# rust-bio/rust-bio

Measured on AMD Instinct MI355X. Metric: GCUPS (SW) + FM-index queries/sec, higher is better.
Workload: dtype int16; 1 GPU; 1000000 x 150 bp synthetic read pairs per GPU, Aligner::local affine-gap (-5,-1,+1,-1), score+coords+traceback ops (BASELINE configs[1]); pairs_per_gpu=1000000, read_len=150, parallelism=shard1

## Files before the change

### rust-bio_amd/csrc/sw_fill_pk16.inc

```
#include <type_traits>

#include "sw_kernels.h"

#ifndef PK16_CELL_KO
#define PK16_CELL_KO 0
#endif

namespace bgsw {
namespace pk16 {

typedef uint32_t pk;

typedef short s16x2 __attribute__((ext_vector_type(2)));
typedef unsigned short u16x2 __attribute__((ext_vector_type(2)));
typedef _Float16 h16x2 __attribute__((ext_vector_type(2)));
__device__ __forceinline__ s16x2 as_s(pk v) { return __builtin_bit_cast(s16x2, v); }
__device__ __forceinline__ u16x2 as_u(pk v) { return __builtin_bit_cast(u16x2, v); }
__device__ __forceinline__ pk bits(s16x2 v) { return __builtin_bit_cast(pk, v); }
__device__ __forceinline__ pk bits(u16x2 v) { return __builtin_bit_cast(pk, v); }
__device__ __forceinline__ pk pk_adds(pk a, pk b) { return bits(__builtin_elementwise_add_sat(as_s(a), as_s(b))); }
__device__ __forceinline__ pk pk_max(pk a, pk b) { return bits(__builtin_elementwise_max(as_s(a), as_s(b))); }
__device__ __forceinline__ pk pk_max3h(pk a, pk b, pk c) {
    const h16x2 x = __builtin_bit_cast(h16x2, a), y = __builtin_bit_cast(h16x2, b), z = __builtin_bit_cast(h16x2, c);
    return __builtin_bit_cast(pk, __builtin_elementwise_maximum(__builtin_elementwise_maximum(x, y), z));
}
__device__ __forceinline__ pk pk_min(pk a, pk b) { return bits(__builtin_elementwise_min(as_s(a), as_s(b))); }
__device__ __forceinline__ pk pk_add_u16(pk a, pk b) { return bits((u16x2)(as_u(a) + as_u(b))); }
__device__ __forceinline__ pk pk_sub_u16(pk a, pk b) { return bits((u16x2)(as_u(a) - as_u(b))); }
__device__ __forceinline__ pk pk_subs_u16(pk a, pk b) { return bits(__builtin_elementwise_sub_sat(as_u(a), as_u(b))); }
__device__ __forceinline__ pk pk_mad_u16(pk a, pk b, pk c) { return bits((u16x2)(as_u(a) * as_u(b) + as_u(c))); }
__device__ __forceinline__ pk dup16(int32_t v) { return ((uint32_t)v & 0xffffu) | ((uint32_t)v << 16); }
__device__ __forceinline__ pk bfi(pk mask, pk a, pk b) { return (a & mask) | (b & ~mask); }
__device__ __forceinline__ pk nz_mask(pk v, pk one) { return pk_sub_u16(pk_subs_u16(one, v), one); }

template <int LP>
__device__ __forceinline__ void scan_first_max(int ll, int64_t& v, uint32_t& idx) {
#pragma unroll
    for (int off = 1; off < LP; off <<= 1) {
        const int64_t ov = __shfl_up(v, off, LP);
        const uint32_t oi = (uint32_t)__shfl_up((int)idx, off, LP);
        if (ll >= off && !(v > ov)) {
            v = ov;
            idx = oi;
        }
    }
}

constexpr int32_t kFloor16 = -2048;

enum { CZ = 0, CF = 1, CI = 2 };
template <int R, int LP, int MODE, int XP, int XS, int YP, int YS, bool LF = false, int FR = 0>
__device__ __forceinline__ void sw_fill_pk16_body(const SwArgs& a) {
    constexpr bool FAST = MODE == 0;
    constexpr int PW = 64 / LP;
    constexpr int NW = tb_words(R);
    constexpr int NH = (R + 2) / 3;
    constexpr bool NARROW = true, LOCAL = XP == CZ && XS == CZ && YP == CZ && YS == CZ;
    constexpr bool ROW0_ZERO = YP == CZ && YS == CZ;
    constexpr int SH = 4;
    constexpr int32_t NEGS = kFloor16 * 16;
    constexpr pk CLEAN = 0xfff0fff0u, FLOORK = 0x80008000u, ONE = 0x00010001u;
    static_assert(LP == 16 || LP == 32, "lanes per pair");
    static_assert(R >= 1 && R <= 12, "rows per lane");
    static_assert(!LF || LOCAL, "LF is a flavour of the local kernel");
    static_assert(FR >= 0 && FR <= 2 && (!FR || LF), "the frame is a cell of the LF flavour");
    (void)NARROW;
    (void)LOCAL;
    constexpr int kTileStride = 20;
    constexpr int kParkDw = 64 * (4 * R + NH + 1), kTileDw = 2 * 64 * kTileStride;
    constexpr int kWaveDw = kParkDw > kTileDw ? kParkDw : kTileDw;
    __shared__ __align__(16) pk s_lds[4 * kWaveDw];
    pk* const wave_lds = s_lds + (threadIdx.x >> 6) * kWaveDw;

    const int lane = threadIdx.x & 63;
    const uint32_t wv = blockIdx.x * (blockDim.x >> 6) + (threadIdx.x >> 6);
    if ((uint64_t)wv * 2 * PW >= a.n_pairs) return;
    if (MODE == 2 && a.len_stats && a.len_stats[0] == a.len_stats[2] && a.len_stats[1] == a.len_stats[3]) return;
    const int g = lane / LP, ll = lane % LP;
    const SwScoring sc = a.sc;
    const SwGeom geo = a.g;
    auto scl = [](int32_t v) -> int32_t { return max(v, kFloor16) * 16; };
    const int32_t go_s = sc.go * 16, xs_s = sc.xs <= kFloor16 ? -(1 << 30) : sc.xs * 16;
    (void)xs_s;
    constexpr int32_t K_XS = C_XS << 1, K_MATCH = C_MATCH << 1, K_SUBST = C_SUBST << 1, K_INS = C_INS << 1,
                      K_DEL = C_DEL << 1, K_XP = C_XP << 1;
    constexpr pk NOFLAG = 0xfffefffeu;
    const pk GE = dup16(sc.ge * 16);
    const pk GOT_I = dup16(sc.go * 16 + K_INS + 1), GOT_D = dup16(sc.go * 16 + K_DEL + 1);
    const pk MISK = dup16((sc.mismatch * 16) | K_SUBST);
    const pk DELTA = dup16(((sc.match * 16) | K_MATCH) - ((sc.mismatch * 16) | K_SUBST));
    const pk XS16 = dup16(scl(sc.xs)), YS16 = dup16(scl(sc.ys));
    const pk XSCAP = sc.xs <= kFloor16 ? FLOORK : 0x7fff7fffu, YSCAP = sc.ys <= kFloor16 ? FLOORK : 0x7fff7fffu;
    (void)XS16; (void)YS16; (void)XSCAP; (void)YSCAP;
    const pk MISC = dup16(-((sc.mismatch * 16) | K_SUBST));
    (void)MISC;
    auto fr = [](int32_t c) -> pk { return (uint32_t)c * 0x10001u; };
    const int32_t gF = -16 * sc.ge, BF = pk16_frame_bias(sc);
    const pk GF = fr(gF);
    const pk KGOI = fr(sc.go * 16 + K_INS + 1 + gF), KGOD = fr(sc.go * 16 + K_DEL + 1 + gF);
    const pk KSUB = fr(((sc.mismatch * 16) | K_SUBST) + 2 * gF);
    const pk KREB = fr(gF * (R - 1));
    (void)GF; (void)KGOI; (void)KGOD; (void)KSUB; (void)KREB;
    constexpr bool DFLOOR = FR == 2 && !(PK16_CELL_KO & 1);
    constexpr bool SYMHI = FR == 2 && !(PK16_CELL_KO & 2);
    constexpr bool ROWMAX2 = FR == 2 && !(PK16_CELL_KO & 4);
    constexpr int SYM_SH = SYMHI ? 8 : 0;
    pk C16 = dup16(16), C32 = dup16(32), C1024 = dup16(1024);
    asm volatile("" : "+s"(C16), "+s"(C32), "+s"(C1024));

    const uint32_t pA = (2 * wv) * PW + g, pB = (2 * wv + 1) * PW + g;
    const bool okA = pA < a.n_pairs, okB = pB < a.n_pairs;
    uint32_t mA = 0, nA = 0, mB = 0, nB = 0;
    uint64_t xoA = 0, yoA = 0, xoB = 0, yoB = 0;
    const uint32_t* perm = a.slot_perm();
    if (okA) {
        const uint64_t r = a.pair0 + (perm ? perm[pA] : pA);
        xoA = a.x_off[r];
        yoA = a.y_off[r];
        mA = (uint32_t)(a.x_off[r + 1] - xoA);
        nA = (uint32_t)(a.y_off[r + 1] - yoA);
        if (len_over(geo, mA, nA)) mA = nA = 0;
    }
    if (okB) {
        const uint64_t r = a.pair0 + (perm ? perm[pB] : pB);
        xoB = a.x_off[r];
        yoB = a.y_off[r];
        mB = (uint32_t)(a.x_off[r + 1] - xoB);
        nB = (uint32_t)(a.y_off[r + 1] - yoB);
        if (len_over(geo, mB, nB)) mB = nB = 0;
    }
    const bool same = okA && okB && mA == mB && nA == nB;
    const bool two = okA && okB && !same;
    const bool m_last0 = LF || __all(!okA || mA % R == 0);
    if (MODE == 0 && !m_last0) return;
    if (MODE == 1 && m_last0) return;
    if (MODE == 2 && !__any(two)) return;
    const uint64_t job_words = tb_job_words(geo.nstrips, geo.nsteps, NW);

    auto do_pass = [&](const int pass) {
        const bool pair_ok = pass == 0 ? okA : two;
        const uint32_t P0 = pass == 0 ? pA : pB, P1 = (pass == 0 && !same) ? pA : pB;
        const uint32_t m = !pair_ok ? 0 : (pass == 0 ? mA : mB), n = !pair_ok ? 0 : (pass == 0 ? nA : nB);
        const uint64_t xs0 = pass == 0 ? xoA : xoB, ys0 = pass == 0 ? yoA : yoB;
        const uint64_t xs1 = (pass == 0 && !same) ? xoA : xoB, ys1 = (pass == 0 && !same) ? yoA : yoB;
        const uint8_t* x0 = a.x + xs0;
        const uint8_t* x1 = a.x + xs1;
        const bool packed = a.packed != 0;
        auto y_pair = [&](uint32_t col) -> pk {
            if (packed) return (sym2(a.y, ys0 + col) | (sym2(a.y, ys1 + col) << 16)) << SYM_SH;
            return ((uint32_t)a.y[ys0 + col] | ((uint32_t)a.y[ys1 + col] << 16)) << SYM_SH;
        };
        const uint32_t Q0 = pair_ok ? P0 : 0, Q1 = pair_ok ? P1 : 0;
        uint32_t* tb0 = (uint32_t*)a.tb + (size_t)(Q0 / PW) * job_words + ((Q0 % PW) * LP + ll) * 16u;
        uint32_t* tb1 = (uint32_t*)a.tb + (size_t)(Q1 / PW) * job_words + ((Q1 % PW) * LP + ll) * 16u;
        int32_t* aux0 = a.aux + (size_t)Q0 * geo.aux_stride;
        int32_t* aux1 = a.aux + (size_t)Q1 * geo.aux_stride;
        int32_t* gLx0 = aux0 + geo.off_Lx();
        int32_t* gLx1 = aux1 + geo.off_Lx();

        uint32_t m_w = m, n_w = n;
#pragma unroll
        for (int o = 32; o; o >>= 1) {
            m_w = max(m_w, (uint32_t)__shfl_xor((int)m_w, o));
            n_w = max(n_w, (uint32_t)__shfl_xor((int)n_w, o));
        }
        (void)m_w;
        n_w = (uint32_t)__builtin_amdgcn_readfirstlane((int)n_w);
        const uint32_t nsteps_w = n_w ? n_w + LP - 1 : 0;

        int32_t fold0;
        uint32_t lx0;
        col0_fold(sc, m, fold0, lx0);
        int32_t Sn0 = sc.ys;
        uint32_t Ly0 = n;
        int32_t S0n = 0;
        uint32_t sb0n = (ROW0_ZERO && n) ? row0_cell(sc, n).sbits : (uint32_t)TB_START;
        if (pair_ok && ll == 0) {
            const int32_t v = m ? (int32_t)col0_cell(sc, m, m, fold0).sbits : (int32_t)TB_START;
            aux0[0] = v;
            aux1[0] = v;
            if (m == 0) {
                if (LP == 16) {
                    *(uint8_t*)gLx0 = (uint8_t)lx0;
                    *(uint8_t*)gLx1 = (uint8_t)lx0;
                } else {
                    *(uint16_t*)gLx0 = (uint16_t)lx0;
                    *(uint16_t*)gLx1 = (uint16_t)lx0;
                }
            }
        }

        const uint32_t rb = (uint32_t)ll * R;
        const int32_t mrow = (int32_t)m - (int32_t)rb - 1;
        pk Sl[R], Dl[R], Il[R], SnR[R], SnB[R], Ly[R], px[R];
        uint64_t nib0S = 0, nib0I = 0;
        uint64_t xw0 = 0, xw1 = 0;
        if (packed && pair_ok && rb < m) {
            const uint32_t* p0 = (const uint32_t*)a.x + ((xs0 + rb) >> 4);
            const uint32_t* p1 = (const uint32_t*)a.x + ((xs1 + rb) >> 4);
            xw0 = (((uint64_t)p0[1] << 32) | p0[0]) >> (2 * ((uint32_t)(xs0 + rb) & 15u));
            xw1 = (((uint64_t)p1[1] << 32) | p1[0]) >> (2 * ((uint32_t)(xs1 + rb) & 15u));
        }
#pragma unroll
        for (int r = 0; r < R; r++) {
            const uint32_t i = rb + r + 1;
            px[r] = 0;
            Sl[r] = Dl[r] = Il[r] = SnR[r] = SnB[r] = FLOORK;
            Ly[r] = 0;
            if (pair_ok && i <= m) {
                px[r] = packed ? (((uint32_t)(xw0 >> (2 * r)) & 3u) | (((uint32_t)(xw1 >> (2 * r)) & 3u) << 16))
                               : ((uint32_t)x0[i - 1] | ((uint32_t)x1[i - 1] << 16));
                px[r] <<= SYM_SH;
                const Col0 c = col0_cell(sc, i, m, fold0);
                Sl[r] = dup16(scl(c.S));
                Il[r] = dup16(scl(c.I) | K_INS);
                nib0S |= (uint64_t)c.sbits << (4 * r);
                nib0I |= (uint64_t)c.ibits << (4 * r);
                if (YS != CI && c.S + sc.ys > NEG) {
                    SnR[r] = dup16(scl(c.S + sc.ys));
                    Ly[r] = dup16((int32_t)n);
                }
            }
        }
        pk diag0 = dup16((pair_ok && rb < m) ? scl(col0_S(sc, rb, m, fold0)) : NEGS);
        if (FR) {
            const int32_t off0 = BF + gF * ((int32_t)ll - 1);
#pragma unroll
            for (int r = 0; r < R; r++) {
                const pk o = fr(off0 + gF * r);
                Sl[r] = (pair_ok && rb + r + 1 <= m) ? Sl[r] + o : o;
                Il[r] += o;
                Dl[r] = 0;
            }
            diag0 = fr(off0 - gF) + ((pair_ok && rb < m) ? dup16(scl(col0_S(sc, rb, m, fold0))) : 0u);
        }

        pk S_out = FLOORK, I_out = FLOORK, cm_out = FLOORK, ca_out = 0, q_out = 0;
        pk ychunk = 0, ychunk_nx = 0;
        pk hwlast[NH];
#pragma unroll
        for (int k = 0; k < NH; k++) hwlast[k] = 0;
        pk lx_n = dup16((int32_t)lx0);
        pk* tileA = wave_lds + (0 * 64 + lane) * kTileStride;
        pk* tileB = wave_lds + (1 * 64 + lane) * kTileStride;
        uint32_t lxaccA = lx0 << (LP == 16 ? 24 : 16), lxaccB = lxaccA;
        if (pair_ok && (uint32_t)ll < n) ychunk_nx = y_pair((uint32_t)ll);

        auto merge_rows = [&](uint32_t blockbase) {
            const pk lybase = dup16((int32_t)(n - blockbase - 16u + (uint32_t)ll));
#pragma unroll
            for (int r = 0; r < R; r++) {
                const pk nr = pk_max(SnR[r], SnB[r] & CLEAN);
                const pk msk = nz_mask(nr ^ SnR[r], ONE);
                Ly[r] = bfi(msk, pk_add_u16(lybase, SnB[r] & 0x000f000fu), Ly[r]);
                SnR[r] = nr;
                SnB[r] = FLOORK;
            }
        };

        constexpr uint32_t tsteps = tb_tile_steps(NW);
        auto store_tile = [&](uint32_t s_any) {
            if (!pair_ok) return;
            const uint32_t off = (s_any / tsteps) * 1024u;
#pragma unroll
            for (int k = 0; k < 4; k++) {
                *(uint4*)&tb0[off + 4 * k] = *(const uint4*)&tileA[4 * k];
                *(uint4*)&tb1[off + 4 * k] = *(const uint4*)&tileB[4 * k];
            }
        };
        uint32_t s_all = pair_ok ? n + (uint32_t)ll : 0u;
#pragma unroll
        for (int o = 32; o; o >>= 1) s_all = min(s_all, (uint32_t)__shfl_xor((int)s_all, o));
        s_all = (uint32_t)__builtin_amdgcn_readfirstlane((int)s_all);
        auto run_steps = [&](auto mr_tag) {
        constexpr int MRk = decltype(mr_tag)::value;
        auto step = [&](auto allon_tag, auto fast_tag, auto trip_tag, const uint32_t s) {
            constexpr bool ALLON = decltype(allon_tag)::value;
            constexpr int TRIP = decltype(trip_tag)::value;
            static_assert(!TRIP || (ALLON && ROWMAX2), "trips are pairs of unpredicated steps of the FR == 2 cell");
            constexpr bool FB = decltype(fast_tag)::value;
            constexpr bool FOLD = XS != CI && !FB;
            if ((s & (LP - 1)) == 0) {
                ychunk = ychunk_nx;
                const uint32_t nb = s + LP + ll;
                if (pair_ok && nb < n) ychunk_nx = y_pair(nb);
            }
            pk S_up = (pk)wave_shr1((int)S_out, (int)S_out), I_up = (pk)wave_shr1((int)I_out, (int)I_out);
            if (FR) {
                S_up -= KREB;
                I_up -= KREB;
            }
            pk cm = FLOORK, ca = 0;
            if (FOLD) {
                cm = (pk)wave_shr1((int)cm_out, (int)cm_out);
                ca = (pk)wave_shr1((int)ca_out, (int)ca_out);
            }
            pk q = (pk)wave_shr1((int)q_out, (int)q_out);
            const uint32_t j = s + 1 - (uint32_t)ll;
            const bool col_ok = ALLON || (pair_ok && (j - 1) < n);
            const pk F0 = fr(BF + gF * (int32_t)s);
            (void)F0;
            if (ll == 0) {
                q = ychunk;
                S_up = FR ? F0 - GF : 0u;
                I_up = FR ? 0u : FLOORK;
                cm = FLOORK;
                ca = 0;
                if (!ROW0_ZERO && col_ok) {
                    const Row0 c = row0_cell(sc, j);
                    int32_t S0 = c.S;
                    uint32_t sb = c.sbits;
                    if (j == n && Sn0 > S0) {
                        S0 = Sn0;
                        sb = TB_YCLIP_SUFFIX;
                    } else if (S0 + sc.ys > Sn0) {
                        Sn0 = S0 + sc.ys;
                        Ly0 = n - j;
                    }
                    S0n = S0;
                    sb0n = sb;
                    S_up = dup16(scl(S0));
                }
            }
            ychunk = (pk)wave_shl1((int)ychunk, (int)ychunk);

            if (col_ok) {
                const pk sprio = dup16((int32_t)(15u - (s & 15u)));
                pk diag = diag0;
                diag0 = S_up;
                pk hw[NH];
                const pk ca_in = ca;
                pk cmk = cm | 0x000f000fu;
                pk snap = cmk;
                pk XKEY = dup16(K_XP);
                if (XP == CF || (XP == CZ && YP != CZ))
                    XKEY = dup16(scl(sc.xp + max(sc.yp, sc.go + sc.ge * ((int32_t)j - 1))) | K_XP);
#pragma unroll
                    for (int r = 0; r < R; r++) {
                        const bool maybe_m = MRk < 0 || r == MRk;
                        const bool is_m = MRk < 0 ? (r == mrow) : (r == MRk && mrow == MRk);
                        const pk e = pk_subs_u16(SYMHI ? DELTA : ONE, px[r] ^ q);
                        const pk Fr = F0 + (uint32_t)r * GF;
                        (void)Fr;
                        pk dk = diag + KSUB;
                        if (SYMHI && !(PK16_CELL_KO & 8)) asm("" : "+v"(dk));
                        const pk m_key = SYMHI   ? e + dk
                                         : FR == 2 ? pk_mad_u16(e, DELTA, diag) + KSUB
                                         : FR    ? pk_max(pk_mad_u16(e, DELTA, diag) + KSUB, Fr)
                                         : LF    ? pk_subs_u16(pk_mad_u16(e, DELTA, diag), MISC)
                                                 : pk_adds(diag, pk_mad_u16(e, DELTA, MISK));
                        const pk Iv_t = FR ? pk_max(I_up, S_up + KGOI) : pk_max(pk_adds(I_up, GE), pk_adds(S_up, GOT_I));
                        const pk Dv_t = DFLOOR ? pk_max3h(Dl[r], Sl[r] + KGOD, Fr)
                                        : FR   ? pk_max(Dl[r], Sl[r] + KGOD)
                                               : pk_max(pk_adds(Dl[r], GE), pk_adds(Sl[r], GOT_D));
                        const pk Iv = Iv_t & NOFLAG, Dv = Dv_t & NOFLAG;
                        pk kb = DFLOOR ? m_key : FR == 2 ? pk_max3h(m_key, Fr, Dv_t) : pk_max(m_key, Dv_t);
                        if (XP != CI && !LF) kb = pk_max(kb, XKEY);
                        kb = DFLOOR ? pk_max3h(kb, Dv_t, Iv_t) : FR == 2 ? pk_max3h(kb, Iv_t, Iv_t) : pk_max(kb, Iv_t);
                        if (FOLD && maybe_m)
                            kb = pk_max(kb, is_m ? ((cmk & CLEAN) | (0x00010001u * K_XS)) : FLOORK);
                        const pk best = kb & CLEAN;
                        const pk best_prev = Sl[r];
                        diag = Sl[r];
                        Sl[r] = best;
                        Dl[r] = Dv;
                        Il[r] = Iv;
                        S_up = best;
                        I_up = Iv;
                        if (FOLD) {
                            if (maybe_m) snap = is_m ? cmk : snap;
                            const pk fv = XS == CZ ? best : pk_min(pk_adds(best, XS16), XSCAP);
                            cmk = pk_max(cmk, fv | (0x00010001u * (uint32_t)(14 - r)));
                        }
                        if (YS != CI) {
                            const pk t1 = YS == CZ ? best : pk_min(pk_adds(best, YS16), YSCAP);
                            if (TRIP == 2)
                                SnB[r] = pk_max3h(SnB[r], best_prev - (Fr - GF - sprio - ONE), best - (Fr - sprio));
                            else if (TRIP == 0)
                                SnB[r] = pk_max(SnB[r], FR ? best - (Fr - sprio) : t1 | sprio);
                        }
                        const pk c5 = pk_mad_u16(Dv_t & ONE, C16, (kb & 0x000e000eu) | (Iv_t & ONE));
                        if (r % 3 == 0)
                            hw[r / 3] = c5;
                        else
                            hw[r / 3] = pk_mad_u16(c5, r % 3 == 1 ? C32 : C1024, hw[r / 3]);
                    }
                if (FOLD) {
                    const pk mbase = dup16(mrow - 14);
                    const pk lo = cmk & 0x000f000fu, slo = snap & 0x000f000fu;
                    if (mrow >= 0 && mrow < R) {
                        const pk is15 = nz_mask(slo ^ 0x000f000fu, ONE);
                        lx_n = bfi(is15, pk_add_u16(slo, mbase), ca_in);
                        if (LP == 16) {
                            lxaccA = __builtin_amdgcn_perm(lx_n, lxaccA, 0x04030201u);
                            lxaccB = __builtin_amdgcn_perm(lx_n, lxaccB, 0x06030201u);
                            if ((j & 3u) == 3u || j == n) {
                                const uint32_t sh = 8u * (3u - (j & 3u));
                                ((uint32_t*)gLx0)[j >> 2] = lxaccA >> sh;
                                ((uint32_t*)gLx1)[j >> 2] = lxaccB >> sh;
                            }
                        } else {
                            lxaccA = __builtin_amdgcn_perm(lx_n, lxaccA, 0x05040302u);
                            lxaccB = __builtin_amdgcn_perm(lx_n, lxaccB, 0x07060302u);
                            if ((j & 1u) == 1u || j == n) {
                                const uint32_t sh = 16u * (1u - (j & 1u));
                                ((uint32_t*)gLx0)[j >> 1] = lxaccA >> sh;
                                ((uint32_t*)gLx1)[j >> 1] = lxaccB >> sh;
                            }
                        }
                    }
                    {
                        const pk is15 = nz_mask(lo ^ 0x000f000fu, ONE);
                        ca = bfi(is15, pk_add_u16(lo, mbase), ca_in);
                    }
                    cm = cmk & CLEAN;
                }
                constexpr pk INV = 0x00010001u * (17u | (17u << 5) | (17u << 10));
                constexpr pk INV_LAST = 0x00010001u * ((R % 3 == 0) ? (17u | (17u << 5) | (17u << 10))
                                                      : (R % 3 == 1) ? 17u : (17u | (17u << 5)));
#pragma unroll
                for (int k = 0; k < NH; k++) {
                    hw[k] ^= (k == NH - 1) ? INV_LAST : INV;
                    hwlast[k] = hw[k];
                }
                const pk h0 = hw[0], h1 = NH > 1 ? hw[NH > 1 ? 1 : 0] : 0u;
                const uint32_t slot = (s % tsteps) * NW;
                if (NW == 1) {
                    tileA[slot] = __builtin_amdgcn_perm(h1, h0, 0x05040100u);
                    tileB[slot] = __builtin_amdgcn_perm(h1, h0, 0x07060302u);
                } else {
                    const pk h2 = hw[NH > 2 ? 2 : 0], h3 = NH > 3 ? hw[NH > 3 ? 3 : 0] : 0u;
                    *(uint2*)&tileA[slot] = make_uint2(__builtin_amdgcn_perm(h1, h0, 0x05040100u),
                                                       __builtin_amdgcn_perm(h3, h2, 0x05040100u));
                    *(uint2*)&tileB[slot] = make_uint2(__builtin_amdgcn_perm(h1, h0, 0x07060302u),
                                                       __builtin_amdgcn_perm(h3, h2, 0x07060302u));
                }
                S_out = S_up;
                I_out = I_up;
                if (FOLD) {
                    cm_out = cm;
                    ca_out = ca;
                }
                q_out = q;
            }
            if (s % tsteps == tsteps - 1) store_tile(s);
            if (YS != CI && (s & 15u) == 15u) merge_rows(s & ~15u);
        };
        uint32_t s = 0;
        const uint32_t s_on = min((uint32_t)(LP - 1), nsteps_w), s_off = max(s_on, min(s_all, nsteps_w));
        constexpr std::false_type no{};
        constexpr std::true_type yes{};
        constexpr std::bool_constant<LF> fast{};
        constexpr std::integral_constant<int, 0> single{};
        constexpr std::integral_constant<int, ROWMAX2 ? 1 : 0> first{};
        constexpr std::integral_constant<int, ROWMAX2 ? 2 : 0> second{};
        for (; s < s_on; s++) step(no, fast, single, s);
        if (ROWMAX2 && (s & 1u) && s < s_off) step(yes, fast, single, s++);
        for (; s + 1 < s_off; s += 2) {
            step(yes, fast, first, s);
            step(yes, fast, second, s + 1);
        }
        for (; s < s_off; s++) step(yes, fast, single, s);
        for (; s < nsteps_w; s++) step(no, fast, single, s);
        };
        run_steps(std::integral_constant<int, (FAST && !LF) ? R - 1 : -1>{});
        if (nsteps_w % tsteps) store_tile(nsteps_w - 1);
        if (YS != CI && nsteps_w) merge_rows((nsteps_w - 1) & ~15u);

        pk* park = wave_lds + lane;
        const pk offl = FR ? fr(BF + gF * ((int32_t)ll + (int32_t)n - 1)) : 0u;
#pragma unroll
        for (int r = 0; r < R; r++) {
            park[(0 * R + r) * 64] = FR ? Sl[r] - (offl + (uint32_t)r * GF) : Sl[r];
            park[(1 * R + r) * 64] = FR ? Il[r] - (offl + (uint32_t)r * GF) : Il[r];
            park[(2 * R + r) * 64] = SnR[r];
            park[(3 * R + r) * 64] = Ly[r];
        }
#pragma unroll
        for (int k = 0; k < NH; k++) park[(4 * R + k) * 64] = hwlast[k];
        park[(4 * R + NH) * 64] = lx_n;
        const int nhalf = (pair_ok && P1 != P0) ? 2 : 1;
        const int nhalf_w = __any(nhalf == 2) ? 2 : 1;
#pragma unroll 1
        for (int h = 0; h < nhalf_w; h++) {
            if (h >= nhalf) continue;
            const uint32_t hs = 16u * (uint32_t)h;
            int32_t* aux = h ? aux1 : aux0;
            int32_t* gLy = aux + geo.off_Ly();
            uint8_t* gBits = (uint8_t*)(aux + geo.off_bits());
            const uint32_t strip = 0;
            struct HalfS {
                const pk* p;
                uint32_t hs;
                __device__ int32_t operator[](int r) const { return (int32_t)(int16_t)(p[r * 64] >> hs); }
            };
            struct HalfU {
                const pk* p;
                uint32_t hs;
                __device__ uint32_t operator[](int r) const { return (p[r * 64] >> hs) & 0xffffu; }
            };
            int32_t Sl_u[R];
#pragma unroll
            for (int r = 0; r < R; r++) Sl_u[r] = (int32_t)(int16_t)(park[r * 64] >> hs);
            const HalfS Il_u{park + 1 * R * 64, hs}, Sn_u{park + 2 * R * 64, hs};
            const HalfU Ly_u{park + 3 * R * 64, hs};
            const uint32_t lx_n_u = (park[(4 * R + NH) * 64] >> hs) & 0xffffu;
            int64_t e_carry = INT64_MIN;
            uint32_t sbf_carry = TB_START, sb2_carry = TB_START;
            int64_t c1v = INT64_MIN, c2v = INT64_MIN;
            uint32_t c1i = 0, c2i = 0;
            auto cell_of = [&](int r) -> uint32_t {
                const uint32_t c = (park[(4 * R + r / 3) * 64] >> (hs + 5 * (r % 3))) & 31u;
                const uint32_t mv = (c >> 1) & 7u;
                return ((LF && mv == 0) ? (uint32_t)C_XP : mv) | ((c & 1u) << 3) | (c & 16u);
            };
            {
                constexpr bool EPI_FOLD_PRE = LF;
                int32_t(&Sl)[R] = Sl_u;
                const HalfS& Il = Il_u;
                const HalfS& Sn = Sn_u;
                const HalfU& Ly = Ly_u;
                const uint32_t lx_n = lx_n_u;
#include "sw_epilogue.inc"
            }
        }
    };
    do_pass(MODE == 2 ? 1 : 0);
}

template <int R, int LP, int XP, int XS, int YP, int YS, bool LF, int FR = 0>
__global__ __launch_bounds__(256) __attribute__((amdgpu_waves_per_eu(R <= 10 ? 3 : 2, R <= 10 ? 3 : 2))) void sw_fill_pk16_kernel(const SwArgs a) {
    sw_fill_pk16_body<R, LP, 0, XP, XS, YP, YS, LF, FR>(a);
}
template <int R, int LP, int XP, int XS, int YP, int YS, bool LF, int FR = 0>
__global__ __launch_bounds__(256) __attribute__((amdgpu_waves_per_eu(R <= 10 ? 3 : 2, R <= 10 ? 3 : 2))) void sw_fill_pk16_rest_kernel(const SwArgs a) {
    sw_fill_pk16_body<R, LP, 1, XP, XS, YP, YS, LF, FR>(a);
}
template <int R, int LP, int XP, int XS, int YP, int YS, bool LF, int FR = 0>
__global__ __launch_bounds__(256) __attribute__((amdgpu_waves_per_eu(R <= 10 ? 3 : 2, R <= 10 ? 3 : 2))) void sw_fill_pk16_second_kernel(const SwArgs a) {
    sw_fill_pk16_body<R, LP, 2, XP, XS, YP, YS, LF, FR>(a);
}

}
}

#define BG_PK16_CASE(LP_, R_)                                                                          \
    if (lp == LP_ && r == R_)                                                                         \
        return which == 0   ? pk16::sw_fill_pk16_kernel<R_, LP_, XP_, XS_, YP_, YS_, LF_, FR_>        \
               : which == 1 ? pk16::sw_fill_pk16_rest_kernel<R_, LP_, XP_, XS_, YP_, YS_, LF_, FR_>   \
                            : pk16::sw_fill_pk16_second_kernel<R_, LP_, XP_, XS_, YP_, YS_, LF_, FR_>;
```

### rust-bio_amd/csrc/sw_traceback.hip

```cpp
#include "sw_kernels.h"

namespace bgsw {

constexpr uint32_t kSegStride = 20;

template <int NW, bool PERM>
__global__ __launch_bounds__(256) __attribute__((amdgpu_waves_per_eu(5, 5))) void sw_traceback_kernel(const SwArgs a) {
    const uint32_t slot = blockIdx.x * blockDim.x + threadIdx.x;
    if (slot >= (a.n_eff ? a.n_eff[PERM ? 1 : 0] : a.n_pairs)) return;
    const uint32_t pair = PERM ? a.perm[slot] : slot;
    const SwScoring sc = a.sc;
    const SwGeom geo = a.g;
    const uint32_t R = geo.r, LP = geo.lp, PW = 64 / geo.lp;

    const uint64_t xo = a.x_off[a.pair0 + pair], yo = a.y_off[a.pair0 + pair];
    const uint32_t m = (uint32_t)(a.x_off[a.pair0 + pair + 1] - xo);
    const uint32_t n = (uint32_t)(a.y_off[a.pair0 + pair + 1] - yo);
    if (len_over(geo, m, n)) {
        bg_alignment_t bad = {};
        bad.xlen = m;
        bad.ylen = n;
        bad.ops_off = (a.pair0 + pair + 1) * a.ops_stride;
        bad.mode = (uint8_t)a.mode;
        bad.status = (int8_t)BG_ERR_INVALID_ARG;
        a.out[a.pair0 + pair] = bad;
        return;
    }

    const int32_t* aux = a.aux + (size_t)slot * geo.aux_stride;
    const int32_t* gLy = aux + geo.off_Ly();
    const int32_t* gLx = aux + geo.off_Lx();
    const uint8_t* bits = (const uint8_t*)(aux + geo.off_bits());
    const uint32_t sbits_m0 = (uint32_t)aux[0];
    const int32_t score = aux[1];
    const uint32_t lxn = (uint32_t)aux[2];

    const uint32_t job = slot / PW, grp = slot % PW;
    const uint32_t* tbj = (const uint32_t*)a.tb + (size_t)job * tb_job_words(geo.nstrips, geo.nsteps, NW);
    __shared__ __align__(16) uint32_t s_seg[256 * kSegStride];
    uint32_t* seg = s_seg + threadIdx.x * kSegStride;
    uint64_t seg_tag = ~0ull;
    auto cell = [&](uint32_t i, uint32_t j) -> uint32_t {
        const uint32_t i1 = i - 1, lrow = __umulhi(i1, geo.r_inv), rr = i1 - lrow * R;
        const uint32_t st = lrow >> geo.lp_shift, llc = lrow & (LP - 1);
        const uint64_t g = (uint64_t)st * geo.nsteps + (j - 1 + llc);
        constexpr uint32_t tsteps = 16 / NW;
        const uint64_t base = (g / tsteps) * 1024ull + (grp * LP + llc) * 16u;
        if (base != seg_tag) {
#pragma unroll
            for (int q = 0; q < 4; q++) *(uint4*)&seg[4 * q] = *(const uint4*)&tbj[base + 4 * q];
            seg_tag = base;
        }
        const uint32_t w = seg[(uint32_t)(g % tsteps) * NW + rr / 6];
        const uint32_t c = rr % 6;
        if (geo.tb_fmt == TBF_K1) return (w >> (5 * c)) & 31u;
        if (geo.tb_fmt == TBF_K1_LF) {
            const uint32_t u = (w >> (5 * c)) & 31u;
            return ((u >> 1) & 7u) | ((~u & 1u) << 3) | (~u & 16u);
        }
        const uint32_t v = (w >> (5 * (c % 3) + 16 * (c / 3))) & 31u;
        const uint32_t mv = (v >> 1) & 7u;
        return ((geo.tb_fmt == TBF_K1P_LF && mv == 0) ? (uint32_t)C_XP : mv) | ((v & 1u) << 3) | (v & 16u);
    };
    auto s_fill = [&](uint32_t i, uint32_t j) -> uint32_t {
        if (j == 0) {
            if (i == 0) return TB_START;
            if (i == m) return sbits_m0;
            return col0_cell(sc, i, m, NEG).sbits;
        }
        if (i == 0) return row0_cell(sc, j).sbits;
        return s_nibble_of_code(cell(i, j) & 7u);
    };
    auto s_nib = [&](uint32_t i, uint32_t j) -> uint32_t {
        if (j == n) return (uint32_t)bits[i] & 15u;
        return s_fill(i, j);
    };
    auto i_nib = [&](uint32_t i, uint32_t j) -> uint32_t {
        if (j == n) return (uint32_t)bits[i] >> 4;
        if (i == 0) return TB_START;
        if (j == 0) return col0_cell(sc, i, m, NEG).ibits;
        return (cell(i, j) & 8u) ? TB_INS : s_fill(i - 1, j);
    };
    auto d_nib = [&](uint32_t i, uint32_t j) -> uint32_t {
        if (j == 0) return TB_START;
        if (i == 0) return row0_cell(sc, j).dbits;
        return (cell(i, j) & 16u) ? TB_DEL : s_fill(i, j - 1);
    };

    uint8_t* ops_end = a.ops ? a.ops + (a.pair0 + pair + 1) * a.ops_stride : nullptr;
    uint32_t n_ops = 0;
    uint32_t clip_len[4] = {0, 0, 0, 0};
    uint32_t n_clips = 0;
    int status = BG_OK;
    const bool dword_ok = ops_end && (((uintptr_t)ops_end & 3) == 0);
    uint32_t acc = 0;
    auto push = [&](uint32_t op) {
        ++n_ops;
        if (!ops_end) return;
        if (dword_ok) {
            acc = (acc << 8) | op;
            if ((n_ops & 3) == 0) *(uint32_t*)(ops_end - n_ops) = acc;
        } else {
            ops_end[-(int64_t)n_ops] = (uint8_t)op;
        }
    };
    auto push_clip = [&](uint32_t op, uint32_t len) {
        if (a.filter_clips) return;
        if (n_clips < 4) clip_len[n_clips] = len;
        else status = BG_ERR_TRACEBACK;
        n_clips++;
        push(op);
    };

    uint32_t i = m, j = n;
    uint32_t xstart = 0, ystart = 0, xend = m, yend = n;
    uint32_t layer = s_nib(m, n);
    const uint32_t guard = 2 * (m + n) + 16;
    uint32_t c_here = 0;
    bool have_c = false;
    for (uint32_t steps = 0; layer != TB_START; steps++) {
        if (steps > guard || (ops_end && n_ops + 1 > a.ops_stride)) {
            status = BG_ERR_TRACEBACK;
            break;
        }
        if (layer >= TB_INS && layer <= TB_MATCH && i >= 1 && i <= m && j >= 1 && j < n) {
            const bool is_ins = layer == TB_INS, is_del = layer == TB_DEL;
            const uint32_t ti = i - (is_del ? 0u : 1u), tj = j - (is_ins ? 0u : 1u);
            if (ti >= 1 && tj >= 1) {
                if (!have_c && (is_ins || is_del)) c_here = cell(i, j);
                const bool ext = (is_ins && (c_here & 8u)) || (is_del && (c_here & 16u));
                push(is_ins ? (uint32_t)BG_OP_INS : is_del ? (uint32_t)BG_OP_DEL : layer == TB_MATCH ? (uint32_t)BG_OP_MATCH : (uint32_t)BG_OP_SUBST);
                c_here = cell(ti, tj);
                have_c = true;
                if (!ext) layer = s_nibble_of_code(c_here & 7u);
                i = ti;
                j = tj;
                continue;
            }
        }
        have_c = false;
        uint32_t next;
        switch (layer) {
            case TB_INS:
                push(BG_OP_INS);
                next = i_nib(i, j);
                i -= 1;
                break;
            case TB_DEL:
                push(BG_OP_DEL);
                next = d_nib(i, j);
                j -= 1;
                break;
            case TB_MATCH:
            case TB_SUBST:
                push(layer == TB_MATCH ? BG_OP_MATCH : BG_OP_SUBST);
                next = (i && j) ? s_nib(i - 1, j - 1) : TB_START;
                i -= 1;
                j -= 1;
                break;
            case TB_XCLIP_PREFIX:
                push_clip(BG_OP_XCLIP, i);
                xstart = i;
                i = 0;
                next = s_nib(0, j);
                break;
            case TB_XCLIP_SUFFIX: {
                if ((geo.tb_fmt == TBF_K1P_LF || geo.tb_fmt == TBF_K1_LF) && j != n) {
                    status = BG_ERR_TRACEBACK;
                    layer = TB_START;
                    continue;
                }
                const uint32_t lx = (j == n) ? lxn
                                    : geo.tb_fmt == TBF_K1 ? (uint32_t)gLx[j]
                                    : geo.lp == 16 ? (uint32_t)((const uint8_t*)gLx)[j] : (uint32_t)((const uint16_t*)gLx)[j];
                push_clip(BG_OP_XCLIP, lx);
                i -= lx;
                xend = i;
                next = i <= m ? s_nib(i, j) : TB_START;
                break;
            }
            case TB_YCLIP_PREFIX:
                push_clip(BG_OP_YCLIP, j);
                ystart = j;
                j = 0;
                next = s_nib(i, 0);
                break;
            default: {
                const uint32_t ly = (uint32_t)gLy[i];
                push_clip(BG_OP_YCLIP, ly);
                j -= ly;
                yend = j;
                next = j <= n ? s_nib(i, j) : TB_START;
                break;
            }
        }
        if (i > m || j > n) {
            status = BG_ERR_TRACEBACK;
            break;
        }
        layer = next;
    }

    if (dword_ok) {
        const uint32_t k = n_ops & 3, done = n_ops - k;
        for (uint32_t t = 0; t < k; t++) ops_end[-(int64_t)(done + t + 1)] = (uint8_t)(acc >> (8 * (k - 1 - t)));
    }
    bg_alignment_t rec;
    rec.score = score;
    rec.xstart = xstart;
    rec.xend = xend;
    rec.ystart = ystart;
    rec.yend = yend;
    rec.xlen = m;
    rec.ylen = n;
    rec.n_ops = n_ops;
    rec.ops_off = (a.pair0 + pair + 1) * a.ops_stride - n_ops;
    const uint32_t nc = n_clips < 4 ? n_clips : 4;
    for (uint32_t c = 0; c < 4; c++) rec.clip_len[c] = c < nc ? clip_len[nc - 1 - c] : 0;
    rec.n_clips = (uint8_t)nc;
    rec.mode = (uint8_t)a.mode;
    rec.status = (int8_t)status;
    rec._pad = 0;
    rec._reserved = 0;
    a.out[a.pair0 + pair] = rec;
}

void launch_traceback(const SwArgs& a, int nw, hipStream_t st) {
    const uint32_t blocks = (a.n_pairs + 255) / 256;
    if (nw == 2)
        sw_traceback_kernel<2, false><<<dim3(blocks), dim3(256), 0, st>>>(a);
    else
        sw_traceback_kernel<1, false><<<dim3(blocks), dim3(256), 0, st>>>(a);
    if (a.perm) {
        if (nw == 2)
            sw_traceback_kernel<2, true><<<dim3(blocks), dim3(256), 0, st>>>(a);
        else
            sw_traceback_kernel<1, true><<<dim3(blocks), dim3(256), 0, st>>>(a);
    }
}

}
```

Measured before the change: 2340 GCUPS.

## Replace serial LF epilogue with wave-parallel DPP first-max reduction

For the LF (local) kernel flavour, the per-half serial epilogue that walked parked rows is replaced by a lane-parallel reduction. Each lane packs candidate scores with row and lane priority bits, and a DPP/shuffle first-max finds the winning lane, which writes only the needed aux and traceback cells. The LDS park area shrinks because the I rows and lx_n are no longer stored. Knock-out macros for setup and epilogue are added for profiling, and traceback gains a guard that rejects reads of last-column cells the new epilogue no longer writes.

New measurement: 2426 GCUPS, median of 6. 1.04x the previous value.

```diff
diff --git a/rust-bio_amd/csrc/sw_fill_pk16.inc b/rust-bio_amd/csrc/sw_fill_pk16.inc
--- a/rust-bio_amd/csrc/sw_fill_pk16.inc
+++ b/rust-bio_amd/csrc/sw_fill_pk16.inc
@@ -44,6 +44,28 @@
             idx = oi;
         }
     }
+}
+
+template <int CTRL>
+__device__ __forceinline__ pk dpp_row(pk v) {
+    return (pk)__builtin_amdgcn_update_dpp((int)v, (int)v, CTRL, 0xf, 0xf, false);
+}
+template <int LP>
+__device__ __forceinline__ pk group_first_max(pk v, int ll, pk& hi) {
+    constexpr pk CLEAN = 0xfff0fff0u, ONE = 0x00010001u;
+    v = pk_max(v, dpp_row<0xb1>(v));
+    v = pk_max(v, dpp_row<0x4e>(v));
+    v = pk_max(v, dpp_row<0x141>(v));
+    v = pk_max(v, dpp_row<0x140>(v));
+    hi = 0;
+    if (LP == 32) {
+        const pk o = (pk)__shfl_xor((int)v, 16);
+        const pk lo_v = ll < 16 ? v : o, up_v = ll < 16 ? o : v;
+        const pk lowwin = nz_mask(pk_max((lo_v & CLEAN) | ONE, up_v & CLEAN) & ONE, ONE);
+        v = bfi(lowwin, lo_v, up_v);
+        hi = ~lowwin & 0x00100010u;
+    }
+    return v;
 }
 
 constexpr int32_t kFloor16 = -2048;
@@ -67,7 +89,7 @@
     (void)NARROW;
     (void)LOCAL;
     constexpr int kTileStride = 20;
-    constexpr int kParkDw = 64 * (4 * R + NH + 1), kTileDw = 2 * 64 * kTileStride;
+    constexpr int kParkDw = LF ? 64 * (3 * R + NH) : 64 * (4 * R + NH + 1), kTileDw = 2 * 64 * kTileStride;
     constexpr int kWaveDw = kParkDw > kTileDw ? kParkDw : kTileDw;
     __shared__ __align__(16) pk s_lds[4 * kWaveDw];
     pk* const wave_lds = s_lds + (threadIdx.x >> 6) * kWaveDw;
@@ -105,6 +127,7 @@
     constexpr bool SYMHI = FR == 2 && !(PK16_CELL_KO & 2);
     constexpr bool ROWMAX2 = FR == 2 && !(PK16_CELL_KO & 4);
     constexpr int SYM_SH = SYMHI ? 8 : 0;
+    constexpr bool KO_EPILOGUE = LF && (PK16_CELL_KO & 16), KO_SETUP = LF && (PK16_CELL_KO & 32);
     pk C16 = dup16(16), C32 = dup16(32), C1024 = dup16(1024);
     asm volatile("" : "+s"(C16), "+s"(C32), "+s"(C1024));
 
@@ -170,7 +193,12 @@
 
         int32_t fold0;
         uint32_t lx0;
-        col0_fold(sc, m, fold0, lx0);
+        if (KO_SETUP) {
+            fold0 = NEG;
+            lx0 = 0;
+        } else {
+            col0_fold(sc, m, fold0, lx0);
+        }
         int32_t Sn0 = sc.ys;
         uint32_t Ly0 = n;
         int32_t S0n = 0;
@@ -211,7 +239,7 @@
                 px[r] = packed ? (((uint32_t)(xw0 >> (2 * r)) & 3u) | (((uint32_t)(xw1 >> (2 * r)) & 3u) << 16))
                                : ((uint32_t)x0[i - 1] | ((uint32_t)x1[i - 1] << 16));
                 px[r] <<= SYM_SH;
-                const Col0 c = col0_cell(sc, i, m, fold0);
+                const Col0 c = KO_SETUP ? Col0{0, kFloor16, (uint32_t)TB_XCLIP_PREFIX, (uint32_t)TB_START} : col0_cell(sc, i, m, fold0);
                 Sl[r] = dup16(scl(c.S));
                 Il[r] = dup16(scl(c.I) | K_INS);
                 nib0S |= (uint64_t)c.sbits << (4 * r);
@@ -222,7 +250,7 @@
                 }
             }
         }
-        pk diag0 = dup16((pair_ok && rb < m) ? scl(col0_S(sc, rb, m, fold0)) : NEGS);
+        pk diag0 = dup16((pair_ok && rb < m) ? (KO_SETUP ? 0 : scl(col0_S(sc, rb, m, fold0))) : NEGS);
         if (FR) {
             const int32_t off0 = BF + gF * ((int32_t)ll - 1);
 #pragma unroll
@@ -232,7 +260,7 @@
                 Il[r] += o;
                 Dl[r] = 0;
             }
-            diag0 = fr(off0 - gF) + ((pair_ok && rb < m) ? dup16(scl(col0_S(sc, rb, m, fold0))) : 0u);
+            diag0 = fr(off0 - gF) + ((pair_ok && rb < m) ? dup16((KO_SETUP ? 0 : scl(col0_S(sc, rb, m, fold0)))) : 0u);
         }
 
         pk S_out = FLOORK, I_out = FLOORK, cm_out = FLOORK, ca_out = 0, q_out = 0;
@@ -466,62 +494,166 @@
         run_steps(std::integral_constant<int, (FAST && !LF) ? R - 1 : -1>{});
         if (nsteps_w % tsteps) store_tile(nsteps_w - 1);
         if (YS != CI && nsteps_w) merge_rows((nsteps_w - 1) & ~15u);
-
-        pk* park = wave_lds + lane;
-        const pk offl = FR ? fr(BF + gF * ((int32_t)ll + (int32_t)n - 1)) : 0u;
-#pragma unroll
-        for (int r = 0; r < R; r++) {
-            park[(0 * R + r) * 64] = FR ? Sl[r] - (offl + (uint32_t)r * GF) : Sl[r];
-            park[(1 * R + r) * 64] = FR ? Il[r] - (offl + (uint32_t)r * GF) : Il[r];
-            park[(2 * R + r) * 64] = SnR[r];
-            park[(3 * R + r) * 64] = Ly[r];
-        }
-#pragma unroll
-        for (int k = 0; k < NH; k++) park[(4 * R + k) * 64] = hwlast[k];
-        park[(4 * R + NH) * 64] = lx_n;
-        const int nhalf = (pair_ok && P1 != P0) ? 2 : 1;
-        const int nhalf_w = __any(nhalf == 2) ? 2 : 1;
+        if (KO_EPILOGUE) {
+#pragma unroll
+            for (int r = 0; r < R; r++) asm volatile("" ::"v"(Sl[r]), "v"(Il[r]), "v"(SnR[r]), "v"(Ly[r]));
+#pragma unroll
+            for (int k = 0; k < NH; k++) asm volatile("" ::"v"(hwlast[k]));
+            asm volatile("" ::"v"(lx_n));
+            return;
+        }
+
+        if constexpr (LF) {
+            const bool nz = n != 0;
+            const int32_t S0fin = nz ? scl(S0n) : 0;
+            const uint32_t sb0fin = nz ? sb0n : (uint32_t)TB_START;
+            const bool has_row0 = pair_ok && ll == 0;
+            pk* park = wave_lds + lane;
+            const pk offl = FR ? fr(BF + gF * ((int32_t)ll + (int32_t)n - 1)) : 0u;
+            pk KF = FLOORK, KC = FLOORK;
+#pragma unroll
+            for (int r = 0; r < R; r++) {
+                const pk sl = FR ? Sl[r] - (offl + (uint32_t)r * GF) : Sl[r];
+                park[(0 * R + r) * 64] = sl;
+                park[(1 * R + r) * 64] = SnR[r];
+                park[(2 * R + r) * 64] = Ly[r];
+                if (r < mrow) {
+                    const pk pr = dup16(14 - r);
+                    KF = pk_max(KF, sl | pr);
+                    KC = pk_max(KC, pk_max(sl, SnR[r]) | pr);
+                }
+            }
+#pragma unroll
+            for (int k = 0; k < NH; k++) park[(3 * R + k) * 64] = hwlast[k];
+            if (has_row0 && m != 0) KC = pk_max(KC, dup16(S0fin) | 0x000f000fu);
+            const pk lprio = dup16(15 - (ll & 15));
+            pk HF, HC;
+            const pk RF = group_first_max<LP>((KF & CLEAN) | lprio, ll, HF), RC = group_first_max<LP>((KC & CLEAN) | lprio, ll, HC);
+            const bool own_m = pair_ok && m != 0 && mrow >= 0 && mrow < R;
+            const bool own_m0 = pair_ok && m == 0 && ll == 0;
+            const int mr = own_m ? mrow : 0;
+            pk Sm = park[(0 * R + mr) * 64], Snm = park[(1 * R + mr) * 64];
+            if (!own_m) {
+                Sm = dup16(S0fin);
+                Snm = FLOORK;
+            }
+            const int ol = m ? (int)((m - 1) / (uint32_t)R) : 0;
+            Sm = (pk)__shfl((int)Sm, ol, LP);
+            Snm = (pk)__shfl((int)Snm, ol, LP);
+            const pk Fs = RF & CLEAN, Cs = RC & CLEAN;
+            const pk v1 = nz ? pk_max(Sm, Fs) : Sm;
+            const pk foldwin = nz ? ~nz_mask(v1 ^ Fs, ONE) : 0u;
+            const pk v2 = pk_max(v1, Cs);
+            const pk c1win = nz_mask(v2 ^ v1, ONE);
+            const pk v3 = pk_max(v2, Snm);
+            const pk ywin = nz_mask(v3 ^ v2, ONE);
+            const pk xswon = foldwin | c1win;
+#pragma unroll
+            for (int h = 0; h < 2; h++) {
+                if (!pair_ok || (h == 1 && P1 == P0)) continue;
+                const uint32_t hs = 16u * (uint32_t)h;
+                int32_t* aux = h ? aux1 : aux0;
+                int32_t* gLy = aux + geo.off_Ly();
+                uint8_t* gBits = (uint8_t*)(aux + geo.off_bits());
+                const bool xs = (xswon >> hs) & 1u, c1 = (c1win >> hs) & 1u, yw = (ywin >> hs) & 1u;
+                auto fillnib = [&](int r) -> uint32_t {
+                    if (!nz) return (uint32_t)(nib0S >> (4 * r)) & 15u;
+                    const uint32_t mv = (park[(3 * R + r / 3) * 64] >> (hs + 5u * (uint32_t)(r % 3) + 1u)) & 7u;
+                    return s_nibble_of_code(mv == 0 ? (uint32_t)C_XP : mv);
+                };
+                const uint32_t wl = 15u - (((c1 ? RC : RF) >> hs) & 15u) + (((c1 ? HC : HF) >> hs) & 16u);
+                if (xs && (uint32_t)ll == wl) {
+                    const uint32_t code = ((c1 ? KC : KF) >> hs) & 15u;
+                    uint32_t istar = 0;
+                    if (code != 15u) {
+                        const int r = min(max(14 - (int)code, 0), R - 1);
+                        istar = rb + (uint32_t)r + 1;
+                        const int32_t sl = (int32_t)(int16_t)(park[(0 * R + r) * 64] >> hs);
+                        const int32_t sn = (int32_t)(int16_t)(park[(1 * R + r) * 64] >> hs);
+                        gBits[istar] = (uint8_t)(sn > sl ? (uint32_t)TB_YCLIP_SUFFIX : fillnib(r));
+                        gLy[istar] = (int32_t)((park[(2 * R + r) * 64] >> hs) & 0xffffu);
+                    }
+                    aux[2] = (int32_t)(m - istar);
+                    aux[3] = (int32_t)istar;
+                }
+                if (own_m || own_m0) {
+                    aux[1] = (int32_t)(int16_t)(v3 >> hs) >> SH;
+                    const uint32_t sbm = yw ? (uint32_t)TB_YCLIP_SUFFIX : xs ? (uint32_t)TB_XCLIP_SUFFIX : own_m ? fillnib(mr) : sb0fin;
+                    gBits[m] = (uint8_t)sbm;
+                    if (own_m) gLy[m] = (int32_t)((park[(2 * R + mr) * 64] >> hs) & 0xffffu);
+                    if (!xs) {
+                        uint32_t istar = m;
+                        if (sbm == (uint32_t)TB_XCLIP_SUFFIX) {
+                            istar = m - lx0;
+                            gBits[istar] = (uint8_t)col0_cell(sc, istar, m, fold0).sbits;
+                            gLy[istar] = (int32_t)n;
+                        }
+                        aux[2] = (int32_t)lx0;
+                        aux[3] = (int32_t)istar;
+                    }
+                }
+                if (has_row0) {
+                    gLy[0] = (int32_t)Ly0;
+                    if (m != 0) gBits[0] = (uint8_t)(sb0fin | (TB_START << 4));
+                }
+            }
+        } else {
+            pk* park = wave_lds + lane;
+            const pk offl = FR ? fr(BF + gF * ((int32_t)ll + (int32_t)n - 1)) : 0u;
+#pragma unroll
+            for (int r = 0; r < R; r++) {
+                park[(0 * R + r) * 64] = FR ? Sl[r] - (offl + (uint32_t)r * GF) : Sl[r];
+                park[(1 * R + r) * 64] = FR ? Il[r] - (offl + (uint32_t)r * GF) : Il[r];
+                park[(2 * R + r) * 64] = SnR[r];
+                park[(3 * R + r) * 64] = Ly[r];
+            }
+#pragma unroll
+            for (int k = 0; k < NH; k++) park[(4 * R + k) * 64] = hwlast[k];
+            park[(4 * R + NH) * 64] = lx_n;
+            const int nhalf = (pair_ok && P1 != P0) ? 2 : 1;
+            const int nhalf_w = __any(nhalf == 2) ? 2 : 1;
 #pragma unroll 1
-        for (int h = 0; h < nhalf_w; h++) {
-            if (h >= nhalf) continue;
-            const uint32_t hs = 16u * (uint32_t)h;
-            int32_t* aux = h ? aux1 : aux0;
-            int32_t* gLy = aux + geo.off_Ly();
-            uint8_t* gBits = (uint8_t*)(aux + geo.off_bits());
-            const uint32_t strip = 0;
-            struct HalfS {
-                const pk* p;
-                uint32_t hs;
-                __device__ int32_t operator[](int r) const { return (int32_t)(int16_t)(p[r * 64] >> hs); }
-            };
-            struct HalfU {
-                const pk* p;
-                uint32_t hs;
-                __device__ uint32_t operator[](int r) const { return (p[r * 64] >> hs) & 0xffffu; }
-            };
-            int32_t Sl_u[R];
-#pragma unroll
-            for (int r = 0; r < R; r++) Sl_u[r] = (int32_t)(int16_t)(park[r * 64] >> hs);
-            const HalfS Il_u{park + 1 * R * 64, hs}, Sn_u{park + 2 * R * 64, hs};
-            const HalfU Ly_u{park + 3 * R * 64, hs};
-            const uint32_t lx_n_u = (park[(4 * R + NH) * 64] >> hs) & 0xffffu;
-            int64_t e_carry = INT64_MIN;
-            uint32_t sbf_carry = TB_START, sb2_carry = TB_START;
-            int64_t c1v = INT64_MIN, c2v = INT64_MIN;
-            uint32_t c1i = 0, c2i = 0;
-            auto cell_of = [&](int r) -> uint32_t {
-                const uint32_t c = (park[(4 * R + r / 3) * 64] >> (hs + 5 * (r % 3))) & 31u;
-                const uint32_t mv = (c >> 1) & 7u;
-                return ((LF && mv == 0) ? (uint32_t)C_XP : mv) | ((c & 1u) << 3) | (c & 16u);
-            };
-            {
-                constexpr bool EPI_FOLD_PRE = LF;
-                int32_t(&Sl)[R] = Sl_u;
-                const HalfS& Il = Il_u;
-                const HalfS& Sn = Sn_u;
-                const HalfU& Ly = Ly_u;
-                const uint32_t lx_n = lx_n_u;
+            for (int h = 0; h < nhalf_w; h++) {
+                if (h >= nhalf) continue;
+                const uint32_t hs = 16u * (uint32_t)h;
+                int32_t* aux = h ? aux1 : aux0;
+                int32_t* gLy = aux + geo.off_Ly();
+                uint8_t* gBits = (uint8_t*)(aux + geo.off_bits());
+                const uint32_t strip = 0;
+                struct HalfS {
+                    const pk* p;
+                    uint32_t hs;
+                    __device__ int32_t operator[](int r) const { return (int32_t)(int16_t)(p[r * 64] >> hs); }
+                };
+                struct HalfU {
+                    const pk* p;
+                    uint32_t hs;
+                    __device__ uint32_t operator[](int r) const { return (p[r * 64] >> hs) & 0xffffu; }
+                };
+                int32_t Sl_u[R];
+#pragma unroll
+                for (int r = 0; r < R; r++) Sl_u[r] = (int32_t)(int16_t)(park[r * 64] >> hs);
+                const HalfS Il_u{park + 1 * R * 64, hs}, Sn_u{park + 2 * R * 64, hs};
+                const HalfU Ly_u{park + 3 * R * 64, hs};
+                const uint32_t lx_n_u = (park[(4 * R + NH) * 64] >> hs) & 0xffffu;
+                int64_t e_carry = INT64_MIN;
+                uint32_t sbf_carry = TB_START, sb2_carry = TB_START;
+                int64_t c1v = INT64_MIN, c2v = INT64_MIN;
+                uint32_t c1i = 0, c2i = 0;
+                auto cell_of = [&](int r) -> uint32_t {
+                    const uint32_t c = (park[(4 * R + r / 3) * 64] >> (hs + 5 * (r % 3))) & 31u;
+                    const uint32_t mv = (c >> 1) & 7u;
+                    return ((LF && mv == 0) ? (uint32_t)C_XP : mv) | ((c & 1u) << 3) | (c & 16u);
+                };
+                {
+                    constexpr bool EPI_FOLD_PRE = false;
+                    int32_t(&Sl)[R] = Sl_u;
+                    const HalfS& Il = Il_u;
+                    const HalfS& Sn = Sn_u;
+                    const HalfU& Ly = Ly_u;
+                    const uint32_t lx_n = lx_n_u;
 #include "sw_epilogue.inc"
+                }
             }
         }
     };
diff --git a/rust-bio_amd/csrc/sw_traceback.hip b/rust-bio_amd/csrc/sw_traceback.hip
--- a/rust-bio_amd/csrc/sw_traceback.hip
+++ b/rust-bio_amd/csrc/sw_traceback.hip
@@ -139,6 +139,14 @@
             }
         }
         have_c = false;
+        if (geo.tb_fmt == TBF_K1P_LF && j == n) {
+            const bool reads_row = layer == TB_XCLIP_SUFFIX || layer == TB_YCLIP_SUFFIX || (layer == TB_YCLIP_PREFIX && n == 0);
+            const uint32_t row = layer == TB_XCLIP_SUFFIX ? i - lxn : i;
+            if (layer == TB_INS || layer == TB_DEL || (reads_row && row <= m && row != 0 && row != m && row != (uint32_t)aux[3])) {
+                status = BG_ERR_TRACEBACK;
+                break;
+            }
+        }
         uint32_t next;
         switch (layer) {
             case TB_INS:
```
